# rag9704/SKIRT

Hardware: AMD Instinct MI355X
Metric: photon packets/sec (whole node), 128^3 octree, 1/2/4/8 MI355X + HBM% (higher is better)
Workload: dtype f64

## Files before the change

### skirt_amd/csrc/device/engine.hip

```cpp
#include <hip/hip_runtime.h>

#include <algorithm>
#include <cfloat>
#include <cmath>
#include <cstring>
#include <string>
#include <type_traits>
#include <vector>

#include "vor_terms.hpp"
#include "cyl2d_walk.hpp"
#include "sph_walk.hpp"
#include "geom_sample.hpp"
#include "polarization.hpp"
#include "../../../include/skirt_mcrt.h"
#include "philox.hpp"

using skirt_dev::PacketRng;

namespace {

constexpr double kDblMax = 1.7976931348623157e308;
constexpr int kBlock = 256;
constexpr int kSegWords = 3 * (kBlock / 64) * 4 / 8;
#ifndef SKIRT_LABS_BUF
#define SKIRT_LABS_BUF 16
#endif
constexpr int kLabsBuf = SKIRT_LABS_BUF;
constexpr int kStepsPerPull = 4;
constexpr int kCtrStride = 32;
enum Ctr : int {
    CTR_RAYS = 0,
    CTR_ACTIVE = 2,
    CTR_PULL = 4,
    CTR_DET = 5,
    CTR_RESERVED = 7,
    CTR_WALK = 8,
    CTR_COUNT = 16
};
constexpr int kCtrWords = CTR_COUNT * kCtrStride;
#define CTR(base, k) ((base)[(k) * kCtrStride])
#define CTRP(base, k) ((base) + (k) * kCtrStride)
constexpr const char* kGeomCapMessage =
    "a TorusGeometry or ConicalShellGeometry found no position in 65536 attempts";
constexpr int kSersicTable = 202;
constexpr int kDetectCopies = 8;
constexpr int kPollEvery = 1;
constexpr int kPollRing = 3;
#ifndef SKIRT_TRACE_WAVES
#define SKIRT_TRACE_WAVES 3
#endif
#define SKIRT_TRACE_ATTR __attribute__((amdgpu_waves_per_eu(SKIRT_TRACE_WAVES)))
#define SKIRT_NOSTORE_TRACE_ATTR __attribute__((amdgpu_waves_per_eu(4)))
#ifndef SKIRT_VOR_TRACE_WAVES
#define SKIRT_VOR_TRACE_WAVES 2
#endif
#define SKIRT_VOR_TRACE_ATTR __attribute__((amdgpu_waves_per_eu(SKIRT_VOR_TRACE_WAVES)))
#ifndef SKIRT_EVENT_WAVES
#define SKIRT_EVENT_WAVES 2
#endif
#define SKIRT_EVENT_ATTR_FOR(GRID, ONECOMP, POL) \
    __attribute__((amdgpu_waves_per_eu(((POL) && !(ONECOMP) && (GRID) == SKIRT_GRID_VORONOI) ? 1 : SKIRT_EVENT_WAVES)))

struct DevInstr {
    int kind, nx, ny, nslots, levels, sedOff;
    int slotStride, stokes;
    long long frameBase;
    long long sedBase;
    double kobs[3];
    double sinphi, cosphi, sintheta, costheta, sinpa, cospa;
    double xpmin, xpsiz, ypmin, ypsiz;
};

enum RayMode : unsigned { RAY_NONE = 0, RAY_PEEL = 1, RAY_FILL = 2, RAY_WALK = 3 };
enum State : int { S_NEW = 0, S_FILL = 2, S_WALK = 3 };
enum PeelCat : unsigned { CAT_STAR_DIRECT = 0, CAT_STAR_SCATTERED = 1, CAT_DUST_DIRECT = 2, CAT_DUST_SCATTERED = 3 };

struct __attribute__((aligned(16))) RayRec {
    double x, y, z;
    double dx, dy, dz;
    double s0;
    double param;
    int idx;
    unsigned flags;
    int ci, cj;
};
static_assert(sizeof(RayRec) == 80, "ray record layout");

struct PathRec {
    double s0, ds, tau0, dtau;
    int m, pad;
};
constexpr int kPathCap = 2048;
constexpr int kContSlots = 1 << 15;
enum ErrorBits : unsigned { ERR_TAU = 1u, ERR_PATH_CAP = 2u, ERR_QUEUE = 4u, ERR_GEOM = 8u };
static_assert(GEOMS_SHELL == SKIRT_GEOM_SHELL && GEOMS_GAMMA == SKIRT_GEOM_GAMMA && GEOMS_GAUSSIAN == SKIRT_GEOM_GAUSSIAN &&
                  GEOMS_TTAURIDISK == SKIRT_GEOM_TTAURIDISK && GEOMS_TORUS == SKIRT_GEOM_TORUS &&
                  GEOMS_CONICALSHELL == SKIRT_GEOM_CONICALSHELL,
              "geom_sample.hpp follows the kinds of skirt_mcrt.h");
template <int GRID>
constexpr bool kEnterInEvent = GRID == SKIRT_GRID_VORONOI;
constexpr int kCellIndexGroup = 2;
constexpr int kNoCell = -2;
constexpr int kOutsideShift = 28;
constexpr int kCellMaskOut = (1 << kOutsideShift) - 1;
template <int GRID>
constexpr int kSegsPerStep = GRID == SKIRT_GRID_VORONOI ? 2 : 1;

struct __attribute__((aligned(16))) DetRec {
    double Lp;
    double tau;
    int l;
    unsigned flags;
};
static_assert(sizeof(DetRec) == 24 || sizeof(DetRec) == 32, "detection record layout");
struct DetPol {
    double Q, U, V;
};
__device__ __forceinline__ unsigned rayMode(unsigned f) { return f & 3u; }
__device__ __forceinline__ unsigned rayCat(unsigned f) { return (f >> 2) & 3u; }
__device__ __forceinline__ int rayInstr(unsigned f) { return (int)((f >> 4) & 63u); }
__device__ __forceinline__ int rayLevel(unsigned f) { return (int)((f >> 10) & 255u); }
__device__ __forceinline__ int rayEll(unsigned f) { return (int)(f >> 18); }

enum FillStatus : int { FILL_TERMINATED = 0, FILL_NO_WALK = 1, FILL_WALK = 2, FILL_FALLBACK = 3 };
__device__ __forceinline__ double fillBiasWeight(double L, double tauint, double taupath, double xi) {
    const double pr = -exp(-tauint) / expm1(-taupath);
    const double q = (1.0 - xi) * pr + xi / taupath;
    return L * (pr / q);
}
template <bool ONECOMP, class Draws>
__device__ __forceinline__ int decideFill(double taupath, double& L, double Lsca, double albedo, double thr, double xi,
                                          Draws& draws, double& tauint) {
    tauint = 0.0;
    if (taupath < 0.0 || isnan(taupath) || isinf(taupath)) return FILL_FALLBACK;
    if (ONECOMP) L = L * albedo * (-expm1(-taupath));
    else L = Lsca;
    if (L <= 0 || L <= thr) return FILL_TERMINATED;
    if (taupath == 0.0) return FILL_NO_WALK;
    const bool biased = xi != 0.0 && draws.biased(xi);
    const double u = draws.uniform();
    double t;
    if (biased || taupath < 1e-10) t = u * taupath;
    else {
        const double norm = 1.0 - exp(-taupath);
        t = -log(1.0 - u * norm);
        if (t > taupath) return FILL_FALLBACK;
    }
    if (xi != 0.0) L = fillBiasWeight(L, t, taupath, xi);
    tauint = t;
    return t > 0 ? FILL_WALK : FILL_NO_WALK;
}
struct FillDrawsStream {
    PacketRng& rng;
    __device__ __forceinline__ bool biased(double xi) { return rng.uniform() < xi; }
    __device__ __forceinline__ double uniform() { return rng.uniform(); }
};
struct FillDrawsAhead {
    bool b;
    double u;
    __device__ __forceinline__ bool biased(double) const { return b; }
    __device__ __forceinline__ double uniform() const { return u; }
};

struct LeafEntry;

struct alignas(16) BlockSite {
    double x, y, z;
    int id, pad;
};
static_assert(sizeof(BlockSite) == 32, "block site layout");

struct alignas(16) VorEntry {
    float ox, oy, oz;
    int next;
};
constexpr int kVorHead = 3;

__device__ __forceinline__ VorEntry vorEntry(const VorEntry* B, int q) {
    const float* P = reinterpret_cast<const float*>(B + kVorHead + (q & ~1));
    const int h = q & 1;
    return VorEntry{P[h], P[2 + h], P[4 + h], __float_as_int(P[6 + h])};
}

// ... 318 lines not shown
        }
    }

    __device__ __forceinline__ void drainStep() {
        constexpr int G = 64 / kLabsBuf;
        const int i = (int)(gstep++ & (kLabsBuf - 1));
        issue(i);
        if (((threadIdx.x & 63) / G) == i) npend = 0;
    }
    __device__ __forceinline__ void drainStep2() {
        constexpr int G = 64 / kLabsBuf;
        const int i = (int)(gstep++ & (kLabsBuf / 2 - 1)) * 2;
        issue(i);
        issue(i + 1);
        const int grp = (threadIdx.x & 63) / G;
        if (grp == i || grp == i + 1) npend = 0;
    }

    __device__ __forceinline__ double rho(int m, int h) const { return a.rho[(size_t)m * a.ncomp + h]; }

    __device__ __forceinline__ bool segment(Ray& r, int m, double rho0, double ds) {
        if (!(ds > 0)) return true;
        double kr = 0.0;
        if (m >= 0) {
            if (ONECOMP) kr = r.kext * rho0;
            else for (int h = 0; h < a.ncomp; h++) kr += sh.kext[h * a.nlambda + r.ell] * rho(m, h);
        }
        const double dtau = kr * ds;
        if (CONT && r.mode == RAY_FILL && m >= 0) {
            const int n = a.pathCnt[r.idx];
            if (n < kPathCap) {
                a.pathBuf[(size_t)r.idx * kPathCap + n] = PathRec{r.s, ds, r.tau, dtau, m, 0};
                a.pathCnt[r.idx] = n + 1;
            } else {
                atomicOr(a.error, ERR_PATH_CAP);
            }
        }
        r.s += ds;
        r.tau += dtau;
        nseg++;
        if (r.mode == RAY_FILL) {
            if (m >= 0 && (!ONECOMP || (STORE && a.store))) {
                double ef;
                if (SKIRT_POLY_EXPM1 && dtau < kCarryTau) ef = oneMinusExpNeg(dtau);
                else ef = -expm1(-dtau);
                const double Lintm = r.param * r.f1 * ef;
                if (dtau < kCarryTau) r.f1 -= r.f1 * ef;
                else r.f1 = exp(-r.tau);
                double albedo;
                if (ONECOMP) albedo = sh.alb[r.ell];
                else {
                    double ksca = 0.0, kext = 0.0;
                    for (int h = 0; h < a.ncomp; h++) {
                        ksca += rho(m, h) * sh.ksca[h * a.nlambda + r.ell];
                        kext += rho(m, h) * sh.kext[h * a.nlambda + r.ell];
                    }
                    albedo = (kext > 0.0) ? ksca / kext : 0.0;
                    r.f2 += albedo * Lintm;
                }
#ifdef SKIRT_DEBUG_FILL
                printf("E S %d %.17g %.17g %.17g\n", m, ds, dtau, (1.0 - albedo) * Lintm);
#endif
                if (STORE && a.store) {
                    pendVal[npend * kBlock + threadIdx.x] = (1.0 - albedo) * Lintm;
                    if (a.labsHi) {
                        const unsigned long long e = (unsigned long long)r.ell * (unsigned)a.labsStride + (unsigned)m;
                        pendIdx[npend * kBlock + threadIdx.x] = (unsigned)e;
                        pendHi[npend * kBlock + threadIdx.x] = (unsigned char)(e >> 32);
                    } else {
                        pendIdx[npend * kBlock + threadIdx.x] = (unsigned)r.ell * (unsigned)a.labsStride + (unsigned)m;
                    }
                    npend++;
                }
            }
        } else if (r.mode == RAY_WALK) {
            if (r.tau > r.param) return false;
            r.f1 = r.tau;
            r.f2 = r.s;
        }
        return true;
    }

    __device__ __forceinline__ void load(Ray& r, unsigned id, bool walkOn) {
        const double2* c = reinterpret_cast<const double2*>(a.rays + id);
        const double2 c0 = c[0], c1 = c[1], c2 = c[2], c3 = c[3];
        const int4 c6 = reinterpret_cast<const int4*>(c)[4];
        r.id = id;
        r.x = c0.x; r.y = c0.y; r.z = c1.x;
        r.dx = c1.y; r.dy = c2.x; r.dz = c2.y;
        r.ix = (fabs(r.dx) > 1e-15) ? 1.0 / r.dx : 0.0;
        r.iy = (fabs(r.dy) > 1e-15) ? 1.0 / r.dy : 0.0;
        r.iz = (fabs(r.dz) > 1e-15) ? 1.0 / r.dz : 0.0;
        r.param = c3.y;
        r.idx = c6.x;
        r.flags = (unsigned)c6.y;
        if (kFuse && walkOn) {
            r.param = fillU(r);
            r.flags = (r.flags & ~3u) | RAY_WALK;
        }
        r.mode = rayMode(r.flags);
        r.ell = rayEll(r.flags);
        r.tau = 0;
        if (CONT && r.mode == RAY_FILL) a.pathCnt[r.idx] = 0;
#ifdef SKIRT_DEBUG_FILL
        if (r.mode == RAY_FILL)
            printf("E L %d %.17g %.17g %.17g %.17g %.17g %.17g %.17g\n", r.ell, r.x, r.y, r.z, r.dx, r.dy, r.dz, r.param);
#endif
        r.s = kEnterInEvent<GRID> ? c3.x : 0.0;
        r.kext = sh.kext[r.ell];
        r.f1 = (r.mode == RAY_FILL) ? 1.0 : 0.0;
        r.f2 = (r.mode == RAY_WALK) ? r.s : 0.0;
        if (kFuse && a.fuse && r.mode == RAY_FILL) {
            fillU(r) = kEnterInEvent<GRID> ? a.fuseU[r.idx] : __hiloint2double(c6.w, c6.z);
            fillThr(r) = kEnterInEvent<GRID> ? a.fuseThr[r.idx] : c3.x;
        }
        nseg = kEnterInEvent<GRID> ? ((unsigned)c6.z >> kOutsideShift) : 0u;
        if (kEnterInEvent<GRID>) {
            r.ci = c6.z & kCellMaskOut;
            r.cj = c6.w;
            r.ck = 0;
        } else if (r.mode != RAY_NONE &&
            !Grid<GRID>::begin(a, sh, r, [&](int m, double rho0, double ds) { return segment(r, m, rho0, ds); })) {
            finish(r);
            r.mode = RAY_NONE;
        }
    }

    __device__ __forceinline__ void finish(Ray& r) {
        atomicAdd(&waveSegs[(threadIdx.x >> 6) * 3 + (r.mode == RAY_FILL ? 0 : r.mode == RAY_WALK ? 1 : 2)], nseg);
        if (a.crossed && r.mode != RAY_WALK) crossedAdd(a, nseg);
        unsigned walkOn = 0;
        double* const walked = (kFuse && a.fuse) ? a.resS : a.resA;
        if (r.mode == RAY_PEEL) {
            a.det[r.idx].tau = r.tau;
        } else if (r.mode == RAY_FILL) {
            a.resA[r.idx] = r.tau;
            if (!ONECOMP) a.resB[r.idx] = r.f2;
            if (kFuse && a.fuse) {
                const double u = fillU(r);
                FillDrawsAhead draws{u < 0.0, fabs(u)};
                double L = r.param, tauint;
                int st = decideFill<ONECOMP>(r.tau, L, r.f2, ONECOMP ? sh.alb[r.ell] : 0.0,
                                              ONECOMP ? r.f2 : fthr, a.xi, draws, tauint);
                if (a.fuse == 2 && (r.idx & 1)) st = FILL_FALLBACK;
                if (st == FILL_WALK) {
                    fillU(r) = tauint;
                    walkOn = kLaneWalkOn | r.id;
                } else {
                    a.resS[r.idx] = -1.0;
                }
            }
        } else {
            const double tauint = r.param;
            double s = 0;
            if (tauint > 0) {
                if (r.tau > tauint) s = r.f2 + ((tauint - r.f1) / (r.tau - r.f1)) * (r.s - r.f2);
                else s = r.f2;
            }
            walked[r.idx] = s;
        }
        r.id = walkOn;
    }
};

#include "detect.hpp"

template <int GRID>
__global__ void __launch_bounds__(kBlock) columnKernel(const Args a, const double* rays, int n, double* out) {
    extern __shared__ __attribute__((aligned(16))) double lds[];
    Shared sh = stageTables(a, lds, gridParts<GRID>());
    const int i = blockIdx.x * blockDim.x + threadIdx.x;
    if (i >= n) return;
// ... 66 lines not shown
        const unsigned long long amask = __ballot(r.mode != RAY_NONE);
        if (imask == 0 && amask == 0) break;
        if (imask != 0 && (amask == 0 || __popcll(imask) >= a.threshold)) {
            const bool walkOn = idle && (r.id & T.kLaneWalkOn) != 0;
            const unsigned long long pmask = imask & ~__ballot(walkOn);
            const unsigned int rank = (unsigned int)__popcll(pmask & ((1ull << lane) - 1ull));
            const unsigned int k = (unsigned int)__popcll(pmask);
            const unsigned int avail = curEnd - cur;
            if (avail < k && !haveNext) { nxt = reserve(); haveNext = true; }
            const unsigned int id = rank < avail ? cur + rank : nxt + (rank - avail);
            if (avail >= k) cur += k;
            else { cur = nxt + (k - avail); curEnd = nxt + kPullChunk; haveNext = false; }
            if (!haveNext && curEnd - cur < kPullChunk / 2 && cur < nrays) { nxt = reserve(); haveNext = true; }
            if (idle) {
                if (!walkOn && id >= nrays) done = true;
                else T.load(r, walkOn ? r.id & ~T.kLaneWalkOn : id < nfront ? id : (unsigned)a.rayCap - 1u - (id - nfront), walkOn);
            }
            __builtin_amdgcn_s_waitcnt(0x0F70);
        }
#pragma unroll 1
        for (int it = 0; it < kStepsPerPull; it++) {
            const unsigned long long live = __ballot(r.mode != RAY_NONE);
            if (live == 0) break;
            T.laneSlots += 64;
            auto seg = [&](int m, double rho0, double ds) { return T.segment(r, m, rho0, ds); };
            if (r.mode != RAY_NONE) {
                if (!Grid<GRID>::step(a, sh, r, seg)) {
                    T.finish(r);
                    r.mode = RAY_NONE;
                }
            }
            if constexpr (!STORE) {
            } else if constexpr (kSegsPerStep<GRID> == 1) {
                T.drainStep();
            } else {
                static_assert(kSegsPerStep<GRID> == 2, "two drains per step hold two adds per step");
                T.drainStep2();
            }
        }
    }
    if constexpr (STORE) T.drain();
    const unsigned* ws = T.waveSegs + (threadIdx.x >> 6) * 3;
    const bool l0 = lane == 0;
    const unsigned long long vals[8] = {0, l0 ? ws[0] : 0u, l0 ? ws[1] : 0u, l0 ? ws[2] : 0u, 0,
                                        l0 ? T.absorbs : 0u, l0 ? T.laneSlots : 0u, l0 ? T.requests : 0u};
    flushStats(a, vals);
}

template <int GRID, bool ONECOMP, bool CONT, bool GLOBAL = false>
__global__ void __launch_bounds__(kBlock) SKIRT_TRACE_ATTR traceKernel(const Args a) {
    traceBody<GRID, ONECOMP, CONT, true, GLOBAL>(a);
}

template <int GRID>
__global__ void __launch_bounds__(kBlock) SKIRT_NOSTORE_TRACE_ATTR traceKernelNoStore(const Args a) {
    traceBody<GRID, true, false, false>(a);
}

template <bool ONECOMP, bool CONT, bool GLOBAL = false>
__global__ void __launch_bounds__(kBlock) SKIRT_VOR_TRACE_ATTR traceKernelVor(const Args a) {
    traceBody<SKIRT_GRID_VORONOI, ONECOMP, CONT, true, GLOBAL>(a);
}

struct Packet {
    double rx, ry, rz, kx, ky, kz, L, Lth;
    int ell, nscatt, stellar, state;
    PacketRng rng;
    PolStokes sv;
};

struct PolDrawsStream {
    PacketRng& rng;
    __device__ __forceinline__ double uniform() { return rng.uniform(); }
};

template <int GRID, bool ONECOMP, bool POL = false>
struct Events {
    const Args& a;
    const Shared& sh;
    unsigned int packets = 0, detects = 0, segFill = 0, segWalk = 0, segPeel = 0;

    __device__ __forceinline__ double rho(int m, int h) const { return a.rho[(size_t)m * a.ncomp + h]; }

    __device__ __forceinline__ bool emitRay(unsigned pos, const Packet& p, double dx, double dy, double dz, double prm,
                                            int idx, unsigned flags, int& vcell) {
        Ray r;
        r.x = p.rx; r.y = p.ry; r.z = p.rz;
        r.dx = dx; r.dy = dy; r.dz = dz;
        r.ix = (fabs(dx) > 1e-15) ? 1.0 / dx : 0.0;
        r.iy = (fabs(dy) > 1e-15) ? 1.0 / dy : 0.0;
        r.iz = (fabs(dz) > 1e-15) ? 1.0 / dz : 0.0;
        r.s = 0;
        r.ci = r.cj = 0;
        const unsigned mode = rayMode(flags);
        int4* dst = reinterpret_cast<int4*>(a.rays + pos);
        bool entered = a.hasDust;
        unsigned nseg = 0;
        if constexpr (kEnterInEvent<GRID>) {
            if (entered) entered = Grid<GRID>::beginAt(a, r, vcell, [&](int, double, double ds) {
                if (ds > 0) { r.s += ds; nseg++; }
                return true;
            });
        }
        if (kEnterInEvent<GRID> && a.crossed && mode != RAY_WALK && a.hasDust) {
            if (!entered) crossedAdd(a, 0);
        }
        if (!entered) {
            if (mode != RAY_PEEL) {
                a.resA[idx] = 0.0;
                if (mode == RAY_WALK && a.fuse) a.resS[idx] = 0.0;
                if (!ONECOMP) a.resB[idx] = 0.0;
                if (mode == RAY_FILL && a.continuous) a.pathCnt[idx] = 0;
            }
            dst[4] = make_int4(idx, (int)RAY_NONE, 0, 0);
            return false;
        }
        double2* d2 = reinterpret_cast<double2*>(dst);
        d2[0] = make_double2(r.x, r.y);
        d2[1] = make_double2(r.z, dx);
        d2[2] = make_double2(dy, dz);
        d2[3] = make_double2(r.s, prm);
        dst[4] = make_int4(idx, (int)flags, r.ci | (int)(min(nseg, 7u) << kOutsideShift), r.cj);
        return true;
    }

    __device__ __forceinline__ void load(int s, Packet& p) const {
        p.rx = a.srx[s]; p.ry = a.sry[s]; p.rz = a.srz[s];
        p.kx = a.skx[s]; p.ky = a.sky[s]; p.kz = a.skz[s];
        p.L = a.sL[s]; p.Lth = a.sLth[s];
        p.ell = a.sell[s]; p.nscatt = a.snscatt[s]; p.stellar = a.sstellar[s]; p.state = a.sstate[s];
        p.rng.k0 = (uint32_t)a.seed; p.rng.k1 = (uint32_t)(a.seed >> 32); p.rng.tag = a.tag;
        p.rng.plo = a.splo[s]; p.rng.phi = a.sphi[s]; p.rng.block = a.sblock[s];
        p.rng.w2 = a.sw2[s]; p.rng.w3 = a.sw3[s]; p.rng.have = a.shave[s];
        if constexpr (POL) {
            p.sv.Q = a.sQ[s]; p.sv.U = a.sU[s]; p.sv.V = a.sV[s];
            p.sv.nx = a.snx[s]; p.sv.ny = a.sny[s]; p.sv.nz = a.snz[s];
            p.sv.pol = a.spol[s];
        }
    }
    __device__ __forceinline__ void store(int s, const Packet& p) const {
        a.srx[s] = p.rx; a.sry[s] = p.ry; a.srz[s] = p.rz;
        a.skx[s] = p.kx; a.sky[s] = p.ky; a.skz[s] = p.kz;
        a.sL[s] = p.L; a.sLth[s] = p.Lth;
        a.sell[s] = p.ell; a.snscatt[s] = p.nscatt; a.sstellar[s] = p.stellar; a.sstate[s] = p.state;
        a.splo[s] = p.rng.plo; a.sphi[s] = p.rng.phi; a.sblock[s] = p.rng.block;
        a.sw2[s] = p.rng.w2; a.sw3[s] = p.rng.w3; a.shave[s] = p.rng.have;
        if constexpr (POL) {
            a.sQ[s] = p.sv.Q; a.sU[s] = p.sv.U; a.sV[s] = p.sv.V;
            a.snx[s] = p.sv.nx; a.sny[s] = p.sv.ny; a.snz[s] = p.sv.nz;
            a.spol[s] = p.sv.pol;
        }
    }

    __device__ __forceinline__ int pixel(const DevInstr& ins, const Packet& p) const {
        const double xpp = -ins.sinphi * p.rx + ins.cosphi * p.ry;
        const double ypp = -ins.cosphi * ins.costheta * p.rx - ins.sinphi * ins.costheta * p.ry + ins.sintheta * p.rz;
        const double xp = ins.cospa * xpp - ins.sinpa * ypp;
        const double yp = ins.sinpa * xpp + ins.cospa * ypp;
        const int i = static_cast<int>(floor((xp - ins.xpmin) / ins.xpsiz));
        const int j = static_cast<int>(floor((yp - ins.ypmin) / ins.ypsiz));
        return (i < 0 || i >= ins.nx || j < 0 || j >= ins.ny) ? -1 : i + ins.nx * j;
    }

    __device__ __forceinline__ bool peelWeight(const DevInstr& ins, const Packet& p, double kx, double ky, double kz,
                                               double& I) const {
        const double cosalpha = kx * ins.kobs[0] + ky * ins.kobs[1] + kz * ins.kobs[2];
        if (ONECOMP) {
            const double g = sh.g[p.ell];
            const double t = 1.0 + g * g - 2 * g * cosalpha;
            I = 0.0 + (1.0 * ((1.0 - g) * (1.0 + g) / sqrt(t * t * t))) * 1.0;
            return true;
        }
        const int m = Grid<GRID>::whichcell(a, sh, p.rx, p.ry, p.rz);
        if (m == -1) return false;
        double sum = 0;
        for (int h = 0; h < a.ncomp; h++) sum += sh.ksca[h * a.nlambda + p.ell] * rho(m, h);
        if (sum <= 0) return false;
        I = 0;
        for (int h = 0; h < a.ncomp; h++) {
            const double wv = sh.ksca[h * a.nlambda + p.ell] * rho(m, h) / sum;
            const double g = sh.g[h * a.nlambda + p.ell];
            const double t = 1.0 + g * g - 2 * g * cosalpha;
            I += (wv * ((1.0 - g) * (1.0 + g) / sqrt(t * t * t))) * 1.0;
        }
        return true;
    }

    __device__ __forceinline__ int peelCell(const Packet& p, int m) const {
        if (m == -1) return -1;
        double sum = 0;
        for (int h = 0; h < a.ncomp; h++) sum += sh.ksca[h * a.nlambda + p.ell] * rho(m, h);
        return sum <= 0 ? -1 : m;
    }

    __device__ __forceinline__ void peelWeightPol(const DevInstr& ins, const Packet& p, int m, double kx, double ky,
                                                  double kz, const PolStokes& sv, double& I, DetPol& q) const {
        const double yx = -ins.cosphi * ins.costheta * ins.cospa - ins.sinphi * ins.sinpa;
        const double yy = -ins.sinphi * ins.costheta * ins.cospa + ins.cosphi * ins.sinpa;
        const double yz = +ins.sintheta * ins.cospa;
        I = 0;
        q.Q = 0; q.U = 0; q.V = 0;
        if (ONECOMP) {
            const PolMix mx = polMixAt(a.polTab, a.ncomp, a.nlambda, a.polNtheta, 0, p.ell);
            polPeelAdd(mx, 1.0, sv, kx, ky, kz, ins.kobs[0], ins.kobs[1], ins.kobs[2], yx, yy, yz, I, q.Q, q.U, q.V);
        } else {
            double sum = 0;
            for (int h = 0; h < a.ncomp; h++) sum += sh.ksca[h * a.nlambda + p.ell] * rho(m, h);
            for (int h = 0; h < a.ncomp; h++) {
                const double wv = sh.ksca[h * a.nlambda + p.ell] * rho(m, h) / sum;
                const PolMix mx = polMixAt(a.polTab, a.ncomp, a.nlambda, a.polNtheta, h, p.ell);
                polPeelAdd(mx, wv, sv, kx, ky, kz, ins.kobs[0], ins.kobs[1], ins.kobs[2], yx, yy, yz, I, q.Q, q.U, q.V);
            }
        }
        polPeelNormalize(I, q.Q, q.U, q.V);
    }

    __device__ __forceinline__ void detectNow(const DevInstr& ins, const Packet& p, double Lp, int l) {
        detects++;
        if (ins.kind != SKIRT_INSTR_FRAME) atomicAddF64(a.tally + ins.sedBase + p.ell, Lp);
        if (l >= 0 && ins.kind != SKIRT_INSTR_SED) atomicAddF64(frameAt(a, ins, p.ell, l, 0), Lp);
    }

    __device__ static double lambertW1(double z) {
        const double eps = 1.0e-12;
        const double em1 = 0.3678794411714423215955237701614608;
        if (z == 0.0) return -kDblMax;
        const double q = z + em1;
// ... 360 lines not shown
    const unsigned int stride = gridDim.x * blockDim.x;
    const unsigned int rounds = (nwork + stride - 1) / stride;
    const unsigned int w0 = blockIdx.x * blockDim.x + threadIdx.x;
    int slotNext = (w0 < nwork) ? (a.init ? (int)w0 : actIn[w0]) : 0;
    for (unsigned int round = 0; round < rounds; round++) {
        const unsigned int w = round * stride + w0;
        const bool valid = w < nwork;
        const int slot = slotNext;
        const unsigned int wn = w + stride;
        if (round + 1 < rounds) slotNext = (wn < nwork) ? (a.init ? (int)wn : actIn[wn]) : 0;
        Packet p;
        p.state = S_NEW;
        double resA = 0.0, resB = 0.0, resS = -1.0;
        int vcell = kNoCell;
        if (valid && !a.init) {
            E.load(slot, p);
            resA = a.resA[slot];
            if (!ONECOMP) resB = a.resB[slot];
            if (a.fuse) {
                resS = a.resS[slot];
                if (p.state == S_WALK) resA = resS;
            }
            if (kEnterInEvent<GRID>) vcell = a.svcell[slot];
        }
        int peel = PEEL_NONE;
        unsigned mainMode = RAY_NONE;
        double mainParam = 0;
        double ox = 0, oy = 0, oz = 0;
        PolStokes osv;
        int pcell = -1;
        if constexpr (POL) polSetUnpolarized(osv);
        if (valid && !a.init) {
            if (p.state == S_FILL) {
                const double taupath = resA;
                FillDrawsStream draws{p.rng};
                double tauint;
                int st = decideFill<ONECOMP>(taupath, p.L, resB, ONECOMP ? sh.alb[p.ell] : 0.0, E.fillThreshold(p), a.xi,
                                             draws, tauint);
                if (st == FILL_FALLBACK) {
                    if (taupath < 0.0 || isnan(taupath) || isinf(taupath)) {
                        atomicOr(a.error, ERR_TAU);
                        st = FILL_TERMINATED;
                    } else {
                        tauint = E.exponCutoffAgain(p, taupath);
                        st = tauint > 0 ? FILL_WALK : FILL_NO_WALK;
                    }
                    resS = -1.0;
                }
                if (st == FILL_TERMINATED) {
                    p.state = S_NEW;
                } else {
                    p.state = S_WALK;
                    if (st == FILL_WALK && resS >= 0.0) resA = resS;
                    else if (st == FILL_WALK) { mainMode = RAY_WALK; mainParam = tauint; }
                    else resA = 0.0;
                }
            }
            if (p.state == S_WALK && mainMode == RAY_NONE) {
                const double s = resA;
                vcell = kNoCell;
                p.rx = p.rx + s * p.kx;
                p.ry = p.ry + s * p.ky;
                p.rz = p.rz + s * p.kz;
                bool ok = a.ninstr > 0 && a.peel && !a.continuous;
                int scell = -1;
                if constexpr (POL) {
                    if (!ONECOMP) {
                        scell = Grid<GRID>::whichcell(a, sh, p.rx, p.ry, p.rz);
                        if (ok) { pcell = E.peelCell(p, scell); ok = pcell >= 0; }
                    }
                    osv = p.sv;
                } else {
                    if (ok && !ONECOMP) { double I; ok = E.peelWeight(sh.instr[0], p, p.kx, p.ky, p.kz, I); }
                }
                if (ok) { peel = PEEL_SCATTER; ox = p.kx; oy = p.ky; oz = p.kz; }
                if constexpr (POL && !ONECOMP) E.scatterIn(p, scell);
                else E.scatter(p);
                mainMode = RAY_FILL;
                mainParam = p.L;
                p.state = S_FILL;
            }
        }
        bool need = valid && p.state == S_NEW && mainMode == RAY_NONE;
        while (__syncthreads_or(need)) {
            unsigned long long* const ctrs[1] = {a.claim};
            const unsigned long long cnt[1] = {need ? 1ull : 0ull};
            unsigned long long res[1];
            blockReserve(ctrs, cnt, res, resv);
            const unsigned long long idx = res[0];
            if (need) {
                if (idx >= total) need = false;
                else if (E.launch(p, globalPacket(a, a.first + idx))) {
                    vcell = kNoCell;
                    if constexpr (POL) polSetUnpolarized(p.sv);
                    if (!(p.L > 0) && !a.crossed) {
                    } else if (a.hasDust) {
                        peel = (a.ninstr > 0 && a.peel) ? PEEL_EMISSION : PEEL_NONE;
                        mainMode = RAY_FILL;
                        mainParam = p.L;
                        p.state = S_FILL;
                        need = false;
                    } else {
                        for (int i = 0; i < a.ninstr; i++) {
                            const DevInstr& ins = sh.instr[i];
                            const int l = ins.kind == SKIRT_INSTR_SED ? -1 : E.pixel(ins, p);
                            if (ins.kind == SKIRT_INSTR_FRAME && l < 0) continue;
                            E.detectNow(ins, p, p.L, l);
                        }
                    }
                }
            }
        }
        int nray = 0;
        if (peel != PEEL_NONE) {
            for (int i = 0; i < a.ninstr; i++) {
                const DevInstr& ins = sh.instr[i];
                if (ins.kind == SKIRT_INSTR_FRAME && E.pixel(ins, p) < 0) continue;
                nray++;
            }
        }
        if (mainMode != RAY_NONE) nray++;
        const bool active = mainMode != RAY_NONE;
        const int npeel = nray - (mainMode != RAY_NONE ? 1 : 0);
        const bool back = a.walkBack && mainMode == RAY_WALK;
        unsigned int pos, apos, dpos, wpos;
        {
            unsigned* const ctrs[4] = {CTRP(a.ctr, CTR_RAYS + a.parity), CTRP(a.ctr, CTR_ACTIVE + (1 - a.parity)),
                                       CTRP(a.ctr, CTR_DET + a.parity), CTRP(a.ctr, CTR_WALK + a.parity)};
            const unsigned cnt[4] = {(unsigned)nray - (back ? 1u : 0u), active ? 1u : 0u, (unsigned)npeel, back ? 1u : 0u};
            unsigned res[4];
            blockReserve(ctrs, cnt, res, resv);
            pos = res[0]; apos = res[1]; dpos = res[2]; wpos = res[3];
        }
        if ((unsigned long long)pos + (unsigned)(nray - (back ? 1 : 0)) > (unsigned long long)a.rayCap ||
            (back && wpos >= (unsigned)a.rayCap) ||
            (unsigned long long)dpos + (unsigned)npeel > (unsigned long long)(a.rayCap - a.nslots)) {
            atomicOr(a.error, ERR_QUEUE);
            nray = 0;
        }
        int inext = 0;
        int fillAt = -1;
        for (int k = 0; k < nray; k++) {
            double dx, dy, dz, prm;
            int idx;
            unsigned flags, at;
            if (k < npeel) {
                int i = inext, l;
                while (true) {
                    const DevInstr& ins = sh.instr[i];
                    l = ins.kind == SKIRT_INSTR_SED ? -1 : E.pixel(ins, p);
                    if (ins.kind == SKIRT_INSTR_FRAME && l < 0) { i++; continue; }
                    break;
                }
                inext = i + 1;
                const DevInstr& ins = sh.instr[i];
                double Lp = p.L;
                unsigned cat, level = 0;
                DetPol dq{0.0, 0.0, 0.0};
                if (peel == PEEL_EMISSION) {
                    cat = p.stellar >= 0 ? CAT_STAR_DIRECT : CAT_DUST_DIRECT;
                } else {
                    double I = 0;
                    if constexpr (POL) E.peelWeightPol(ins, p, pcell, ox, oy, oz, osv, I, dq);
                    else E.peelWeight(ins, p, ox, oy, oz, I);
                    Lp = p.L * I;
                    cat = p.stellar >= 0 ? CAT_STAR_SCATTERED : CAT_DUST_SCATTERED;
                    level = (unsigned)min(p.nscatt, 255);
                }
                dx = ins.kobs[0]; dy = ins.kobs[1]; dz = ins.kobs[2];
                prm = Lp;
                flags = RAY_PEEL | (cat << 2) | ((unsigned)i << 4) | (level << 10) | ((unsigned)p.ell << 18);
                idx = (int)(dpos + k);
                a.det[idx] = DetRec{Lp, 0.0, l, flags};
                if constexpr (POL) a.detPol[idx] = dq;
                at = pos++;
            } else {
                dx = p.kx; dy = p.ky; dz = p.kz;
                prm = mainParam;
                idx = slot;
                flags = mainMode | ((unsigned)p.ell << 18);
                at = back ? (unsigned)a.rayCap - 1u - wpos : pos++;
            }
            const bool in = E.emitRay(at, p, dx, dy, dz, prm, idx, flags, vcell);
            if (k >= npeel && in && mainMode == RAY_FILL) fillAt = (int)at;
        }
        if (active) actOut[apos] = slot;
        if (valid) E.store(slot, p);
        if (kEnterInEvent<GRID> && valid) a.svcell[slot] = vcell;
        if (a.fuse && fillAt >= 0) {
            PacketRng ahead = p.rng;
            const bool biased = a.xi != 0.0 && ahead.uniform() < a.xi;
            const double u = ahead.uniform();
            const double fu = biased ? -u : u, fthr = E.fillThreshold(p);
            RayRec* rec = a.rays + fillAt;
            if (kEnterInEvent<GRID>) {
                a.fuseU[slot] = fu;
                a.fuseThr[slot] = fthr;
            } else {
                rec->s0 = fthr;
                rec->ci = __double2loint(fu);
                rec->cj = __double2hiint(fu);
            }
        }
    }
    const unsigned long long vals[8] = {E.packets, E.segFill, E.segWalk, E.segPeel, E.detects, 0, 0, 0};
    flushStats(a, vals);
}

template <int GRID, bool ONECOMP>
__global__ void __launch_bounds__(kBlock) contKernel(const Args a) {
    __shared__ unsigned long long resv[2 * (kBlock / 64) + 2];
    extern __shared__ __attribute__((aligned(16))) double lds[];
    const unsigned int nwork = CTR(a.ctr, CTR_ACTIVE + a.parity);
    if (nwork == 0) return;
    Shared sh = stageTables(a, lds, gridParts<GRID>() | STAGE_OPTICS | STAGE_INSTR);
    Events<GRID, ONECOMP> E{a, sh};
    const int* actIn = a.act[a.parity];
    const unsigned int stride = gridDim.x * blockDim.x;
    const unsigned int rounds = (nwork + stride - 1) / stride;
    const int Nl = a.nlambda;
    for (unsigned int round = 0; round < rounds; round++) {
        const unsigned int w = round * stride + blockIdx.x * blockDim.x + threadIdx.x;
        const int slot = w < nwork ? actIn[w] : 0;
        Packet p;
        p.state = S_NEW;
        if (w < nwork) E.load(slot, p);
        const bool fill = w < nwork && p.state == S_FILL;
        const int nrec = fill ? a.pathCnt[slot] : 0;
        const PathRec* rec = a.pathBuf + (size_t)slot * kPathCap;
        auto weights = [&](int m, double* wv, double& albedo) {
            double ksca = 0.0, kext = 0.0;
            for (int h = 0; h < a.ncomp; h++) {
                const double rho = a.rho[(size_t)m * a.ncomp + h];
                wv[h] = rho * sh.ksca[h * Nl + p.ell];
                ksca += rho * sh.ksca[h * Nl + p.ell];
                kext += rho * sh.kext[h * Nl + p.ell];
            }
            if (!(ksca > 0.0)) return false;
            for (int h = 0; h < a.ncomp; h++) wv[h] /= ksca;
            albedo = ksca / kext;
            return true;
        };
        const PacketRng rng0 = p.rng;
        unsigned int nray = 0;
        for (int n = 0; n < nrec; n++) {
            double wv[8], albedo;
            if (!weights(rec[n].m, wv, albedo)) continue;
            const double s = rec[n].s0 + p.rng.uniform() * rec[n].ds;
            Packet q = p;
            q.rx = p.rx + s * p.kx; q.ry = p.ry + s * p.ky; q.rz = p.rz + s * p.kz;
            for (int i = 0; i < a.ninstr; i++)
                if (!(sh.instr[i].kind == SKIRT_INSTR_FRAME && E.pixel(sh.instr[i], q) < 0)) nray++;
        }
        unsigned* const ctrs[2] = {CTRP(a.ctr, CTR_RAYS + a.parity), CTRP(a.ctr, CTR_DET + a.parity)};
        const unsigned cnt[2] = {nray, nray};
        unsigned res[2];
        blockReserve(ctrs, cnt, res, resv);
        unsigned int pos = res[0], dpos = res[1];
        if (nray && (pos + nray > (unsigned)a.rayCap || dpos + nray > (unsigned)(a.rayCap - a.nslots))) {
            atomicOr(a.error, ERR_QUEUE);
            nray = 0;
        }
        if (nray) {
            PacketRng rng = rng0;
            for (int n = 0; n < nrec; n++) {
                double wv[8], albedo;
                if (!weights(rec[n].m, wv, albedo)) continue;
                const double factorm = albedo * exp(-rec[n].tau0) * (-expm1(-rec[n].dtau));
                const double s = rec[n].s0 + rng.uniform() * rec[n].ds;
                Packet q = p;
                q.rx = p.rx + s * p.kx; q.ry = p.ry + s * p.ky; q.rz = p.rz + s * p.kz;
                int qcell = kNoCell;
                for (int i = 0; i < a.ninstr; i++) {
                    const DevInstr& ins = sh.instr[i];
                    const int l = ins.kind == SKIRT_INSTR_SED ? -1 : E.pixel(ins, q);
                    if (ins.kind == SKIRT_INSTR_FRAME && l < 0) continue;
                    const double cosalpha = p.kx * ins.kobs[0] + p.ky * ins.kobs[1] + p.kz * ins.kobs[2];
                    double I = 0;
                    for (int h = 0; h < a.ncomp; h++) {
                        const double g = sh.g[h * Nl + p.ell];
                        const double t = 1.0 + g * g - 2 * g * cosalpha;
                        const double wgt = wv[h] * ((1.0 - g) * (1.0 + g) / sqrt(t * t * t));
                        I += wgt * 1.0;
                    }
                    const double Lp = p.L * (factorm * I);
                    const unsigned cat = p.stellar >= 0 ? CAT_STAR_SCATTERED : CAT_DUST_SCATTERED;
                    const unsigned level = (unsigned)min(p.nscatt + 1, 255);
                    const unsigned flags = RAY_PEEL | (cat << 2) | ((unsigned)i << 4) | (level << 10) | ((unsigned)p.ell << 18);
                    a.det[dpos] = DetRec{Lp, 0.0, l, flags};
                    E.emitRay(pos++, q, ins.kobs[0], ins.kobs[1], ins.kobs[2], Lp, (int)dpos, flags, qcell);
                    dpos++;
                }
            }
        }
        if (fill) {
            a.sblock[slot] = p.rng.block; a.sw2[slot] = p.rng.w2; a.sw3[slot] = p.rng.w3; a.shave[slot] = p.rng.have;
        }
    }
    const unsigned long long vals[8] = {0, E.segFill, E.segWalk, E.segPeel, 0, 0, 0, 0};
    flushStats(a, vals);
}

}


struct SkirtMcrt {
    int device = 0;
    hipStream_t own = nullptr, stream = nullptr;
    hipEvent_t ev0 = nullptr, ev1 = nullptr;
    std::string err;
    int gridKind = -1, ncells = 0, nx = 0, ny = 0, nz = 0, nnodes = 0, search = 1;
    int ndev = 0;
    int labsStride = 0;
    bool brick = false;
    double eps = 0, gx0 = 0, gx1 = 0, gy0 = 0, gy1 = 0, gz0 = 0, gz1 = 0;
    double* dMesh = nullptr;
    double* dBox = nullptr;
    int *dFirstChild = nullptr, *dCellnumber = nullptr, *dNbrOffset = nullptr, *dNbrList = nullptr;
    signed char* dSplitDir = nullptr;
    int* dFather = nullptr;
    bool binTree = false;
    double *dSite = nullptr, *dCellBbox = nullptr;
    VorEntry* dVorSlots = nullptr;
    int *dVorStart = nullptr, *dBlockOffset = nullptr;
    BlockSite* dBlockSites = nullptr;
    std::vector<VorEntry> vorSlotsHost;
    std::vector<int> vorStartHost;
    double vorScale = 1.0;
    int vnb = 0;
    int mapL = -1, mapN = 0;
    double mapInv[3] = {0, 0, 0};
    double mapOrigin[3] = {0, 0, 0};
    double* dTreeT = nullptr;
    LeafEntry* dLeafMap = nullptr;
    bool mapReady = false;
    int lastWalk = -1;
    std::vector<int> devCell;
    int ncomp = 0, nlambda = 0;
    double *dRho = nullptr, *dOptics = nullptr;
    double* dPolTab = nullptr;
    std::vector<double> polTab;
    int polNtheta = 0;
    int nstar = 0;
    double *dGeomParam = nullptr, *dLum = nullptr, *dLumtot = nullptr, *dCdf = nullptr;
    int lumLo = 0, lumHi = -1;
    double* dGeomTable = nullptr;
    double emissionBias = 0.5;
    double *dCellLv = nullptr, *dCellCdf = nullptr, *dCellLtot = nullptr;
    int* dCellGuide = nullptr;
    size_t cellGuideCount = 0;
    double cellBias = 0.5;
    int* dCellNode = nullptr;
    double* dLabsDust = nullptr;
    bool ownLabsDust = true;
    double* dLabsRep = nullptr;
    size_t labsRepBytes = 0;
    bool labsRepDirty = false;
    int emisNtemp = 0;
    double *dEmisVolume = nullptr, *dEmisKabs = nullptr, *dEmisSigma = nullptr, *dEmisMu = nullptr, *dEmisTv = nullptr,
           *dEmisPlanck = nullptr, *dEmisLambda = nullptr, *dEmisDlambda = nullptr, *dEmisScratch = nullptr;
    int* dDevCell = nullptr;
    std::vector<DevInstr> instr;
    DevInstr* dInstr = nullptr;
    size_t nInstrTally = 0;
    int nsed = 0;
    double *dLabs = nullptr, *dTally = nullptr;
    bool ownLabs = true, ownTally = true;
    unsigned long long *dClaim = nullptr, *dStats = nullptr;
    unsigned long long* dCrossed = nullptr;
    int crossedBins = 0;
    unsigned int *dError = nullptr, *dCtr = nullptr, *hCtr = nullptr;
    hipStream_t sD = nullptr;
    hipEvent_t evDetT = nullptr, evDet[2] = {}, evDetJoin = nullptr;
    std::vector<hipEvent_t> pollEv;
    int nslots = 0, rayCap = 0;
    bool poolPath = false;
    bool poolDetPair = false;
    bool poolPol = false;
    void* dPool = nullptr;
    size_t poolBytes = 0;
    int traceGrid = 0, threshold = 0, slotsWanted = 0;
    int walkBack = getenv("SKIRT_AMD_WALK_BACK") ? atoi(getenv("SKIRT_AMD_WALK_BACK")) : -1;
    int fuseWalk = getenv("SKIRT_AMD_FUSE_WALK") ? atoi(getenv("SKIRT_AMD_FUSE_WALK")) : -1;
    int traceBlocksPerCU = 0;
    int lastDetCopies = 0;
    double lastMs = 0;
    bool phaseTimed = false;
    std::vector<hipEvent_t> traceEv;
    int traceLaunches = 0;
    uint64_t packagesTotal = 0;
    double traceMs = 0;
    uint64_t traceLaunchesTotal = 0;
    int numCUs = 0;
    size_t ldsMax = 64 * 1024;
    int lastIterations = 0;
    SkirtReduceTallyFn reduce = nullptr;
    void* reduceUser = nullptr;
    bool instrReduced = false;
};

namespace {

int fail(SkirtMcrt* c, int code, const std::string& msg) {
    if (c) c->err = msg;
    return code;
}

#define HIPCHECK(ctx, call)                                                                    \
    do {                                                                                       \
        hipError_t e_ = (call);                                                                \
        if (e_ != hipSuccess) return fail(ctx, SKIRT_ERR_HIP, std::string(#call) + ": " + hipGetErrorString(e_)); \
    } while (0)

template <class T>
int upload(SkirtMcrt* c, T*& dst, const T* src, size_t n) {
    if (dst) { (void)hipFree(dst); dst = nullptr; }
    if (n == 0) return SKIRT_OK;
    if (!src) return fail(c, SKIRT_ERR_ARG, "null host array");
    HIPCHECK(c, hipMalloc(&dst, n * sizeof(T)));
    HIPCHECK(c, hipMemcpy(dst, src, n * sizeof(T), hipMemcpyHostToDevice));
    return SKIRT_OK;
}

struct Walk {
    int kind, stat;
    bool meshInLds;
};
constexpr Walk kWalks[] = {
    {SKIRT_GRID_CARTESIAN, SKIRT_WALK_CARTESIAN, true},
    {SKIRT_GRID_OCTREE, SKIRT_WALK_OCTREE_MAP, false},
    {kBinTreeMap, SKIRT_WALK_KDTREE_MAP, false},
    {kOctreeBookkeeping, SKIRT_WALK_OCTREE_BOOKKEEPING, false},
    {SKIRT_GRID_CYLINDER2D, SKIRT_WALK_CYLINDER2D, true},
    {SKIRT_GRID_SPHERE1D, SKIRT_WALK_SPHERE1D, true},
    {SKIRT_GRID_SPHERE2D, SKIRT_WALK_SPHERE2D, true},
    {SKIRT_GRID_VORONOI, SKIRT_WALK_VORONOI, false},
    {kOctreeNodes, SKIRT_WALK_TREE_NODES, false},
};
constexpr int kNumWalks = (int)(sizeof kWalks / sizeof kWalks[0]);

const Walk& walkOf(int kind) {
    for (const Walk& w : kWalks)
        if (w.kind == kind) return w;
    return kWalks[kNumWalks - 1];
}

template <int I = 0, class F>
auto withWalk(int kind, F&& f) {
    if constexpr (I + 1 < kNumWalks) {
        if (kind == kWalks[I].kind) return f(std::integral_constant<int, kWalks[I].kind>{});
        return withWalk<I + 1>(kind, f);
    } else {
        return f(std::integral_constant<int, kWalks[I].kind>{});
    }
}

template <class F>
auto withBool(bool b, F&& f) {
    return b ? f(std::true_type{}) : f(std::false_type{});
}

int walkKind(const SkirtMcrt* c, bool hasDust) {
    if (c->gridKind < 0) return kOctreeNodes;
    if (c->gridKind != SKIRT_GRID_OCTREE) return c->gridKind;
    if (c->search == SKIRT_TREE_BOOKKEEPING) return kOctreeBookkeeping;
    if (c->mapL >= 0 && hasDust) return c->binTree ? kBinTreeMap : SKIRT_GRID_OCTREE;
    return kOctreeNodes;
}

const void* traceKernelOf(int kind, bool one, bool continuous, bool global, bool noStore) {
    return withWalk(kind, [&](auto g) {
        constexpr int G = decltype(g)::value;
        if constexpr (G != SKIRT_GRID_VORONOI)
            if (noStore) return (const void*)traceKernelNoStore<G>;
        return withBool(global, [&](auto gl) {
            constexpr bool L = decltype(gl)::value;
            if constexpr (G == SKIRT_GRID_VORONOI) {
                if (!continuous) return one ? (const void*)traceKernelVor<true, false, L> : (const void*)traceKernelVor<false, false, L>;
                return one ? (const void*)traceKernelVor<true, true, L> : (const void*)traceKernelVor<false, true, L>;
            } else {
                if (!continuous) return one ? (const void*)traceKernel<G, true, false, L> : (const void*)traceKernel<G, false, false, L>;
                return one ? (const void*)traceKernel<G, true, true, L> : (const void*)traceKernel<G, false, true, L>;
            }
        });
    });
}

static_assert(sizeof(RayRec) % 16 == 0 && alignof(RayRec) == 16 && sizeof(DetRec) % 16 == 0 && alignof(DetRec) == 16 &&
                  alignof(PathRec) <= 16,
              "pool order: ray records, detection records, 8-byte arrays, 4-byte arrays, aligned path records");
constexpr size_t kPoolSpare = 4096;
size_t poolLayout(char* base, size_t nslots, size_t rayCap, bool detPair, bool path, bool pol, Args& a) {
    char* p = base;
    size_t bytes = 0;
    auto take = [&](auto*& d, size_t count) {
        using T = std::remove_reference_t<decltype(*d)>;
        d = reinterpret_cast<T*>(p);
        if (base) p += count * sizeof(T);
        bytes += count * sizeof(T);
    };
    take(a.rays, rayCap);
    take(a.det, (detPair ? 2 : 1) * (rayCap - nslots));
    for (double** d : {&a.srx, &a.sry, &a.srz, &a.skx, &a.sky, &a.skz, &a.sL, &a.sLth, &a.resA, &a.resB, &a.resS, &a.fuseU,
                       &a.fuseThr})
        take(*d, nslots);
    a.detPol = nullptr;
    a.sQ = a.sU = a.sV = a.snx = a.sny = a.snz = nullptr;
    a.spol = nullptr;
    if (pol) {
        take(a.detPol, (detPair ? 2 : 1) * (rayCap - nslots));
        for (double** d : {&a.sQ, &a.sU, &a.sV, &a.snx, &a.sny, &a.snz}) take(*d, nslots);
        take(a.spol, nslots);
    }
    for (int** d : {&a.sell, &a.snscatt, &a.sstellar, &a.sstate, &a.svcell}) take(*d, nslots);
    for (uint32_t** d : {&a.splo, &a.sphi, &a.sblock, &a.sw2, &a.sw3, &a.shave}) take(*d, nslots);
    take(a.act[0], nslots);
    take(a.act[1], nslots);
    a.pathBuf = nullptr;
    a.pathCnt = nullptr;
    if (path) {
        p = reinterpret_cast<char*>(((uintptr_t)p + 15) & ~(uintptr_t)15);
        take(a.pathBuf, nslots * kPathCap);
        take(a.pathCnt, nslots);
    }
    return bytes;
}

int ensurePool(SkirtMcrt* c, int nslots, bool continuous, bool detPair, bool pol) {
    const int ninstr = (int)c->instr.size();
    const size_t rays = (size_t)nslots * (1 + ninstr) + (continuous ? (size_t)nslots * kPathCap * ninstr : 0);
    if (rays >= (size_t)INT32_MAX) return fail(c, SKIRT_ERR_UNSUPPORTED, "ray queue too large");
    const int rayCap = (int)rays;
    const bool path = continuous && nslots > 0;
    if (c->dPool && c->nslots == nslots && c->rayCap == rayCap && c->poolPath == path && c->poolDetPair == detPair &&
        c->poolPol == pol)
        return SKIRT_OK;
    Args counted{};
    const size_t bytes = poolLayout(nullptr, (size_t)nslots, (size_t)rayCap, detPair, path, pol, counted) + kPoolSpare;
    c->poolPath = path;
    c->poolPol = pol;
    c->poolDetPair = detPair;
    if (c->dPool) { (void)hipFree(c->dPool); c->dPool = nullptr; }
    HIPCHECK(c, hipMalloc(&c->dPool, bytes));
    c->poolBytes = bytes;
    c->nslots = nslots;
    c->rayCap = rayCap;
    return SKIRT_OK;
}

void carvePool(SkirtMcrt* c, Args& a) {
    poolLayout(static_cast<char*>(c->dPool), (size_t)c->nslots, (size_t)c->rayCap, c->poolDetPair, c->poolPath, c->poolPol, a);
    a.nslots = c->nslots;
    a.rayCap = c->rayCap;
    a.ctr = c->dCtr;
}

int planLeafMap(SkirtMcrt* c, const SkirtGridDesc* g) {
    c->mapL = -1;
    c->mapReady = false;
    if (c->dLeafMap) { (void)hipFree(c->dLeafMap); c->dLeafMap = nullptr; }
    const char* env = getenv("SKIRT_AMD_LEAFMAP");
    if (env && env[0] == '0') return SKIRT_OK;
    const bool bin = g->split_dir != nullptr;
    if (c->ndev >= (int)(1u << (bin ? kBinCellBits : kLeafLevelShift))) return SKIRT_OK;
    const int maxL = bin ? kMaxBinMapLevel : kMaxMapLevel;
    struct Item { int node, lv[3], idx[3]; };
    std::vector<Item> stack{{0, {0, 0, 0}, {0, 0, 0}}};
    std::vector<Item> nodes;
    nodes.reserve(g->nnodes);
    int L = 0;
    while (!stack.empty()) {
        const Item it = stack.back();
        stack.pop_back();
        nodes.push_back(it);
        L = std::max(L, std::max(it.lv[0], std::max(it.lv[1], it.lv[2])));
        if (L > maxL) return SKIRT_OK;
        const int fc = g->first_child[it.node];
        if (fc < 0) continue;
        if (bin) {
            const int d = g->split_dir[it.node];
            for (int k = 0; k < 2; k++) {
                Item ch = it;
                ch.node = fc + k;
                ch.lv[d]++;
                ch.idx[d] = 2 * it.idx[d] + k;
                stack.push_back(ch);
            }
        } else {
            for (int k = 0; k < 8; k++) {
                Item ch;
                ch.node = fc + k;
                for (int ax = 0; ax < 3; ax++) {
                    ch.lv[ax] = it.lv[ax] + 1;
                    ch.idx[ax] = 2 * it.idx[ax] + ((k >> ax) & 1);
                }
                stack.push_back(ch);
            }
        }
    }
    if ((int)nodes.size() != g->nnodes) return SKIRT_OK;
    const int N = 1 << L;
    std::vector<double> T(3 * (size_t)(N + 1));
    for (int ax = 0; ax < 3; ax++) {
        double* t = T.data() + ax * (N + 1);
        t[0] = g->box[ax];
        t[N] = g->box[3 + ax];
        for (int w = N; w > 1; w >>= 1)
            for (int lo = 0; lo < N; lo += w) t[lo + w / 2] = 0.5 * (t[lo] + t[lo + w]);
        for (int j = 0; j < N; j++)
            if (!(t[j] < t[j + 1])) return SKIRT_OK;
    }
    for (const Item& it : nodes) {
        const double* b = g->box + 6 * (size_t)it.node;
        for (int ax = 0; ax < 3; ax++) {
            const int sh = L - it.lv[ax];
            const double* t = T.data() + ax * (N + 1);
            if (b[ax] != t[it.idx[ax] << sh] || b[3 + ax] != t[(it.idx[ax] + 1) << sh]) return SKIRT_OK;
        }
    }
    int rc = upload(c, c->dTreeT, T.data(), T.size());
    if (rc) return rc;
    c->mapL = L;
    c->mapN = N;
    for (int ax = 0; ax < 3; ax++) c->mapInv[ax] = N / (g->box[3 + ax] - g->box[ax]);
    for (int ax = 0; ax < 3; ax++) c->mapOrigin[ax] = T[ax * (N + 1)];
    return SKIRT_OK;
}

void gridArgs(const SkirtMcrt* c, Args& a) {
    a.ncells = c->ncells;
    a.labsStride = c->labsStride;
    a.nx = c->nx; a.ny = c->ny; a.nz = c->nz;
    a.brick = c->brick ? 1 : 0;
    a.mesh = c->dMesh;
// ... 1544 lines not shown
```

Measured before the change: 244.2 million.

## Replace 80-byte ray records with 16-byte slot references for non-Voronoi grids

For non-Voronoi, non-continuous runs the ray queue now stores a 16-byte reference (index, flags, packet slot) instead of a full 80-byte ray record. The walk kernel rebuilds position, direction and parameters from the per-slot packet arrays or the instrument direction for peel rays. Fuse parameters always go to the per-slot arrays, and packet stores skip fields that only change on launch. This cuts HBM write and read traffic for the ray queue at the cost of scattered per-slot gathers in the walker. It also relies on slot state staying consistent between the event and walk kernels.

New measurement: 248.8 million, median of 6. +1.9%, better.

```diff
diff --git a/skirt_amd/csrc/device/engine.hip b/skirt_amd/csrc/device/engine.hip
--- a/skirt_amd/csrc/device/engine.hip
+++ b/skirt_amd/csrc/device/engine.hip
@@ -76,6 +76,13 @@
 enum State : int { S_NEW = 0, S_FILL = 2, S_WALK = 3 };
 enum PeelCat : unsigned { CAT_STAR_DIRECT = 0, CAT_STAR_SCATTERED = 1, CAT_DUST_DIRECT = 2, CAT_DUST_SCATTERED = 3 };
 
+struct __attribute__((aligned(16))) RayRef {
+    int idx;
+    unsigned flags;
+    int slot;
+    int spare;
+};
+static_assert(sizeof(RayRef) == 16, "ray reference layout");
 struct __attribute__((aligned(16))) RayRec {
     double x, y, z;
     double dx, dy, dz;
@@ -100,6 +107,8 @@
               "geom_sample.hpp follows the kinds of skirt_mcrt.h");
 template <int GRID>
 constexpr bool kEnterInEvent = GRID == SKIRT_GRID_VORONOI;
+template <int GRID, bool CONT>
+constexpr bool kRayRefs = !kEnterInEvent<GRID> && !CONT;
 constexpr int kCellIndexGroup = 2;
 constexpr int kNoCell = -2;
 constexpr int kOutsideShift = 28;
@@ -584,12 +593,33 @@
     }
 
     __device__ __forceinline__ void load(Ray& r, unsigned id, bool walkOn) {
-        const double2* c = reinterpret_cast<const double2*>(a.rays + id);
-        const double2 c0 = c[0], c1 = c[1], c2 = c[2], c3 = c[3];
-        const int4 c6 = reinterpret_cast<const int4*>(c)[4];
+        double2 c3;
+        int4 c6;
         r.id = id;
-        r.x = c0.x; r.y = c0.y; r.z = c1.x;
-        r.dx = c1.y; r.dy = c2.x; r.dz = c2.y;
+        if constexpr (kRayRefs<GRID, CONT>) {
+            const int4 q = reinterpret_cast<const int4*>(a.rays)[id];
+            const int slot = q.z;
+            unsigned flags = (unsigned)q.y;
+            if (kFuse && walkOn) flags = (flags & ~3u) | RAY_WALK;
+            const bool peel = rayMode(flags) == RAY_PEEL;
+            const double* kobs = a.instr[peel ? rayInstr(flags) : 0].kobs;
+            const double* const px = peel ? kobs : a.skx + slot;
+            const double* const py = peel ? kobs + 1 : a.sky + slot;
+            const double* const pz = peel ? kobs + 2 : a.skz + slot;
+            r.x = a.srx[slot]; r.y = a.sry[slot]; r.z = a.srz[slot];
+            r.dx = *px; r.dy = *py; r.dz = *pz;
+            double L = a.sL[slot], u = a.fuseU[slot], thr = a.fuseThr[slot];
+            asm volatile("" : "+v"(L), "+v"(u), "+v"(thr));
+            c3 = make_double2(thr, rayMode(flags) == RAY_WALK ? u : L);
+            c6 = make_int4(q.x, (int)flags, __double2loint(u), __double2hiint(u));
+        } else {
+            const double2* c = reinterpret_cast<const double2*>(a.rays + id);
+            const double2 c0 = c[0], c1 = c[1], c2 = c[2];
+            c3 = c[3];
+            c6 = reinterpret_cast<const int4*>(c)[4];
+            r.x = c0.x; r.y = c0.y; r.z = c1.x;
+            r.dx = c1.y; r.dy = c2.x; r.dz = c2.y;
+        }
         r.ix = (fabs(r.dx) > 1e-15) ? 1.0 / r.dx : 0.0;
         r.iy = (fabs(r.dy) > 1e-15) ? 1.0 / r.dy : 0.0;
         r.iz = (fabs(r.dz) > 1e-15) ? 1.0 / r.dz : 0.0;
@@ -822,8 +852,25 @@
 
     __device__ __forceinline__ double rho(int m, int h) const { return a.rho[(size_t)m * a.ncomp + h]; }
 
+    __device__ __forceinline__ bool rayRefs() const { return !kEnterInEvent<GRID> && (POL || !a.continuous); }
+
     __device__ __forceinline__ bool emitRay(unsigned pos, const Packet& p, double dx, double dy, double dz, double prm,
-                                            int idx, unsigned flags, int& vcell) {
+                                            int idx, unsigned flags, int& vcell, int slot) {
+        if (rayRefs()) {
+            int4* const ref = reinterpret_cast<int4*>(a.rays) + pos;
+            const unsigned mode = rayMode(flags);
+            if (!a.hasDust) {
+                if (mode != RAY_PEEL) {
+                    a.resA[idx] = 0.0;
+                    if (mode == RAY_WALK && a.fuse) a.resS[idx] = 0.0;
+                    if (!ONECOMP) a.resB[idx] = 0.0;
+                }
+                *ref = make_int4(idx, (int)RAY_NONE, slot, 0);
+                return false;
+            }
+            *ref = make_int4(idx, (int)flags, slot, 0);
+            return true;
+        }
         Ray r;
         r.x = p.rx; r.y = p.ry; r.z = p.rz;
         r.dx = dx; r.dy = dy; r.dz = dz;
@@ -878,11 +925,12 @@
             p.sv.pol = a.spol[s];
         }
     }
-    __device__ __forceinline__ void store(int s, const Packet& p) const {
+    __device__ __forceinline__ void store(int s, const Packet& p, bool fresh) const {
         a.srx[s] = p.rx; a.sry[s] = p.ry; a.srz[s] = p.rz;
         a.skx[s] = p.kx; a.sky[s] = p.ky; a.skz[s] = p.kz;
-        a.sL[s] = p.L; a.sLth[s] = p.Lth;
-        a.sell[s] = p.ell; a.snscatt[s] = p.nscatt; a.sstellar[s] = p.stellar; a.sstate[s] = p.state;
+        a.sL[s] = p.L;
+        if (fresh) { a.sLth[s] = p.Lth; a.sell[s] = p.ell; a.sstellar[s] = p.stellar; }
+        a.snscatt[s] = p.nscatt; a.sstate[s] = p.state;
         a.splo[s] = p.rng.plo; a.sphi[s] = p.rng.phi; a.sblock[s] = p.rng.block;
         a.sw2[s] = p.rng.w2; a.sw3[s] = p.rng.w3; a.shave[s] = p.rng.have;
         if constexpr (POL) {
@@ -1409,6 +1457,7 @@
             }
         }
         bool need = valid && p.state == S_NEW && mainMode == RAY_NONE;
+        bool fresh = false;
         while (__syncthreads_or(need)) {
             unsigned long long* const ctrs[1] = {a.claim};
             const unsigned long long cnt[1] = {need ? 1ull : 0ull};
@@ -1419,6 +1468,7 @@
                 if (idx >= total) need = false;
                 else if (E.launch(p, globalPacket(a, a.first + idx))) {
                     vcell = kNoCell;
+                    fresh = true;
                     if constexpr (POL) polSetUnpolarized(p.sv);
                     if (!(p.L > 0) && !a.crossed) {
                     } else if (a.hasDust) {
@@ -1508,26 +1558,20 @@
                 flags = mainMode | ((unsigned)p.ell << 18);
                 at = back ? (unsigned)a.rayCap - 1u - wpos : pos++;
             }
-            const bool in = E.emitRay(at, p, dx, dy, dz, prm, idx, flags, vcell);
+            const bool in = E.emitRay(at, p, dx, dy, dz, prm, idx, flags, vcell, slot);
             if (k >= npeel && in && mainMode == RAY_FILL) fillAt = (int)at;
         }
         if (active) actOut[apos] = slot;
-        if (valid) E.store(slot, p);
+        if (valid) E.store(slot, p, fresh);
+        if (E.rayRefs() && mainMode == RAY_WALK) a.fuseU[slot] = mainParam;
         if (kEnterInEvent<GRID> && valid) a.svcell[slot] = vcell;
         if (a.fuse && fillAt >= 0) {
             PacketRng ahead = p.rng;
             const bool biased = a.xi != 0.0 && ahead.uniform() < a.xi;
             const double u = ahead.uniform();
             const double fu = biased ? -u : u, fthr = E.fillThreshold(p);
-            RayRec* rec = a.rays + fillAt;
-            if (kEnterInEvent<GRID>) {
-                a.fuseU[slot] = fu;
-                a.fuseThr[slot] = fthr;
-            } else {
-                rec->s0 = fthr;
-                rec->ci = __double2loint(fu);
-                rec->cj = __double2hiint(fu);
-            }
+            a.fuseU[slot] = fu;
+            a.fuseThr[slot] = fthr;
         }
     }
     const unsigned long long vals[8] = {E.packets, E.segFill, E.segWalk, E.segPeel, E.detects, 0, 0, 0};
@@ -1615,7 +1659,7 @@
                     const unsigned level = (unsigned)min(p.nscatt + 1, 255);
                     const unsigned flags = RAY_PEEL | (cat << 2) | ((unsigned)i << 4) | (level << 10) | ((unsigned)p.ell << 18);
                     a.det[dpos] = DetRec{Lp, 0.0, l, flags};
-                    E.emitRay(pos++, q, ins.kobs[0], ins.kobs[1], ins.kobs[2], Lp, (int)dpos, flags, qcell);
+                    E.emitRay(pos++, q, ins.kobs[0], ins.kobs[1], ins.kobs[2], Lp, (int)dpos, flags, qcell, slot);
                     dpos++;
                 }
             }
@@ -1701,6 +1745,7 @@
     hipEvent_t evDetT = nullptr, evDet[2] = {}, evDetJoin = nullptr;
     std::vector<hipEvent_t> pollEv;
     int nslots = 0, rayCap = 0;
+    bool poolRefs = false;
     bool poolPath = false;
     bool poolDetPair = false;
     bool poolPol = false;
@@ -1813,11 +1858,11 @@
     });
 }
 
-static_assert(sizeof(RayRec) % 16 == 0 && alignof(RayRec) == 16 && sizeof(DetRec) % 16 == 0 && alignof(DetRec) == 16 &&
-                  alignof(PathRec) <= 16,
+static_assert(sizeof(RayRec) % 16 == 0 && alignof(RayRec) == 16 && sizeof(RayRef) % 16 == 0 && alignof(RayRef) == 16 &&
+                  sizeof(DetRec) % 16 == 0 && alignof(DetRec) == 16 && alignof(PathRec) <= 16,
               "pool order: ray records, detection records, 8-byte arrays, 4-byte arrays, aligned path records");
 constexpr size_t kPoolSpare = 4096;
-size_t poolLayout(char* base, size_t nslots, size_t rayCap, bool detPair, bool path, bool pol, Args& a) {
+size_t poolLayout(char* base, size_t nslots, size_t rayCap, bool refs, bool detPair, bool path, bool pol, Args& a) {
     char* p = base;
     size_t bytes = 0;
     auto take = [&](auto*& d, size_t count) {
@@ -1826,7 +1871,13 @@
         if (base) p += count * sizeof(T);
         bytes += count * sizeof(T);
     };
-    take(a.rays, rayCap);
+    if (refs) {
+        RayRef* queue = nullptr;
+        take(queue, rayCap);
+        a.rays = reinterpret_cast<RayRec*>(queue);
+    } else {
+        take(a.rays, rayCap);
+    }
     take(a.det, (detPair ? 2 : 1) * (rayCap - nslots));
     for (double** d : {&a.srx, &a.sry, &a.srz, &a.skx, &a.sky, &a.skz, &a.sL, &a.sLth, &a.resA, &a.resB, &a.resS, &a.fuseU,
                        &a.fuseThr})
@@ -1859,11 +1910,13 @@
     if (rays >= (size_t)INT32_MAX) return fail(c, SKIRT_ERR_UNSUPPORTED, "ray queue too large");
     const int rayCap = (int)rays;
     const bool path = continuous && nslots > 0;
-    if (c->dPool && c->nslots == nslots && c->rayCap == rayCap && c->poolPath == path && c->poolDetPair == detPair &&
-        c->poolPol == pol)
+    const bool refs = !continuous && c->gridKind != SKIRT_GRID_VORONOI;
+    if (c->dPool && c->nslots == nslots && c->rayCap == rayCap && c->poolRefs == refs && c->poolPath == path &&
+        c->poolDetPair == detPair && c->poolPol == pol)
         return SKIRT_OK;
     Args counted{};
-    const size_t bytes = poolLayout(nullptr, (size_t)nslots, (size_t)rayCap, detPair, path, pol, counted) + kPoolSpare;
+    const size_t bytes = poolLayout(nullptr, (size_t)nslots, (size_t)rayCap, refs, detPair, path, pol, counted) + kPoolSpare;
+    c->poolRefs = refs;
     c->poolPath = path;
     c->poolPol = pol;
     c->poolDetPair = detPair;
@@ -1876,7 +1929,8 @@
 }
 
 void carvePool(SkirtMcrt* c, Args& a) {
-    poolLayout(static_cast<char*>(c->dPool), (size_t)c->nslots, (size_t)c->rayCap, c->poolDetPair, c->poolPath, c->poolPol, a);
+    poolLayout(static_cast<char*>(c->dPool), (size_t)c->nslots, (size_t)c->rayCap, c->poolRefs, c->poolDetPair, c->poolPath,
+               c->poolPol, a);
     a.nslots = c->nslots;
     a.rayCap = c->rayCap;
     a.ctr = c->dCtr;
```
